# theivyzhang/droplet_visual_odometry

Measured on AMD Instinct MI355X. Metric: frames/sec (detect+match+pose) at 1280×720, 2000 feats; ATE vs reference, higher is better.
Workload: dtype u8/f32/f64

## Files before the change

### droplet_visual_odometry_amd/csrc/match.hip

```cpp
#include <algorithm>
#include <cfloat>
#include <climits>

#include "dvo_internal.h"

namespace dvo {
namespace {

typedef int v4i __attribute__((ext_vector_type(4)));
typedef int v8i __attribute__((ext_vector_type(8)));
typedef float v16f __attribute__((ext_vector_type(16)));
constexpr int kMWaves = 4, kMQB = 64 * kMWaves, kMStage = 64;
constexpr int kKeyBase = 1 << 20;

constexpr int kMChunks = 8;
constexpr int kMKs = 4;
typedef v16f acc_t;
__device__ __forceinline__ v4i expand_chunk(uint32_t bits, uint32_t base) {
    v4i r;
#pragma unroll
    for (int k = 0; k < 4; ++k) {
        const uint32_t L = (((bits >> (8 * k)) & 0xFu) * 0x00204081u) & 0x01010101u;
        const uint32_t H = (((bits >> (8 * k + 4)) & 0xFu) * 0x00204081u) & 0x01010101u;
        r[k] = (int)(base ^ (L << 3) ^ (H << 7));
    }
    return r;
}
constexpr uint32_t kExpQ = 0xAAAAAAAAu, kExpT = 0x22222222u;
__device__ __forceinline__ acc_t mfma_chunk(v4i a, v4i b, acc_t c) {
    const v8i A = {a[0], a[1], a[2], a[3], 0, 0, 0, 0}, B = {b[0], b[1], b[2], b[3], 0, 0, 0, 0};
    return __builtin_amdgcn_mfma_scale_f32_32x32x64_f8f6f4(A, B, c, 4, 4, 0, 0x7F7F7F7F, 0, 0x8B8B8B8B);
}
__device__ __forceinline__ int key_add(float a, float c) { return __float_as_int(a + c); }
__device__ __forceinline__ int key_value(int kbits) { return (int)__int_as_float(kbits); }
constexpr int kKeyNone = 0x7F000000;
constexpr int kChunkMask = kMChunks - 1;
__device__ __forceinline__ int key_old(int k) { return ((k >> 13) << 16) | (k & 8191); }

template <bool kFull>
__device__ __forceinline__ void nn_stage(const v4i* btc, int* cmin, const v4i (&A)[2][kMKs], int (&best)[2][16], int t0,
                                         int nt, int r, int h, int rowb, int nq) {
    const float rbf = (float)rowb;
    acc_t rb0, rb1;
#pragma unroll
    for (int g = 0; g < 16; ++g) {
        const int goff = (g & 3) + 8 * (g >> 2);
        rb0[g] = rbf + (float)goff;
        rb1[g] = rbf + (float)(32 + goff);
    }
#pragma unroll 1
    for (int tt = 0; tt < kMStage / 32; ++tt) {
        const int j = t0 + 32 * tt + r;
        const float cf = (float)(j < nt ? j : (1 << 30));
        acc_t acc0 = rb0, acc1 = rb1;
#pragma unroll
        for (int ks = 0; ks < kMKs; ++ks) {
            const v4i B = btc[(32 * tt + r) * kMChunks + ((2 * ks + h) ^ (r & kChunkMask))];
            acc0 = mfma_chunk(A[0][ks], B, acc0);
            acc1 = mfma_chunk(A[1][ks], B, acc1);
        }
        int cm = 0x7FFFFFFF;
#pragma unroll
        for (int g = 0; g < 16; ++g) {
            const int goff = (g & 3) + 8 * (g >> 2);
            best[0][g] = min(best[0][g], key_add(acc0[g], cf));
            best[1][g] = min(best[1][g], key_add(acc1[g], cf));
            int k0 = __float_as_int(acc0[g]), k1 = __float_as_int(acc1[g]);
            if (!kFull) {
                k0 = rowb - kKeyBase + goff < nq ? k0 : kKeyNone;
                k1 = rowb - kKeyBase + 32 + goff < nq ? k1 : kKeyNone;
            }
            cm = min(cm, min(k0, k1));
        }
        if (j < nt) atomicMin(&cmin[32 * tt + r], cm);
    }
}

struct NnOperands {
    const uint8_t* q0;
    const uint8_t* t0;
    int64_t stride;
    int nq_fix, nt_fix;
};

#ifndef DVO_MATCH_WAVES
#define DVO_MATCH_WAVES 1
#endif
__global__ __launch_bounds__(256) __attribute__((amdgpu_waves_per_eu(DVO_MATCH_WAVES)))
void nn_mfma_kernel(StreamParams P, NnOperands O, int pairs, int nqb, int tsplit) {
    __shared__ v4i bt[2][kMStage * kMChunks];
    __shared__ int colmin[2][kMStage];
    const int nwg = gridDim.x;
    const int L0 = (blockIdx.x & 7) * (nwg >> 3) + (blockIdx.x >> 3);
    const int L = L0 / tsplit, ts = L0 - L * tsplit;
    const int p = L / nqb, qb = L - p * nqb;
    if (p >= pairs) return;
    const int cap = P.plan.kp_cap;
    const int fp = pair_frame(P, p);
    const int nq = O.nq_fix >= 0 ? O.nq_fix : min(P.buf.nkp[fp], cap);
    const int nt = O.nt_fix >= 0 ? O.nt_fix : min(P.buf.nkp[fp + 1], cap);
    const int qbase = qb * kMQB;
    if (qbase >= nq) return;
    const int lane = threadIdx.x & 63, wid = threadIdx.x >> 6;
    const int r = lane & 31, h = lane >> 5;
    const uint4* XQ = reinterpret_cast<const uint4*>(O.q0 + fp * O.stride);
    const uint2* XT = reinterpret_cast<const uint2*>(O.t0 + fp * O.stride);
    int32_t* fwd = P.buf.nn + (int64_t)p * cap;
    int32_t* bwd = P.buf.nn + ((int64_t)P.nframes + p) * cap;
    const int qs = qbase + wid * 64;
    v4i A[2][kMKs];
    int best[2][16];
#pragma unroll
    for (int s2 = 0; s2 < 2; ++s2) {
        const int q = qs + 32 * s2 + r;
        const uint4 w0 = q < nq ? XQ[2 * (int64_t)q] : make_uint4(0, 0, 0, 0);
        const uint4 w1 = q < nq ? XQ[2 * (int64_t)q + 1] : make_uint4(0, 0, 0, 0);
        const uint32_t wd[8] = {w0.x, w0.y, w0.z, w0.w, w1.x, w1.y, w1.z, w1.w};
#pragma unroll
        for (int ks = 0; ks < kMKs; ++ks) {
            const int ch = 2 * ks + h;
            const uint32_t bits = wd[ch];
            A[s2][ks] = q < nq ? expand_chunk(bits, kExpQ) : (v4i){0, 0, 0, 0};
        }
#pragma unroll
        for (int g = 0; g < 16; ++g) best[s2][g] = 0x7FFFFFFF;
    }
    const int rowb = kKeyBase + qs + 4 * h;
    const bool full = qs + 64 <= nq;
    const int nst_all = (nt + kMStage - 1) / kMStage;
    const int st0 = (int)((int64_t)nst_all * ts / tsplit), nst = (int)((int64_t)nst_all * (ts + 1) / tsplit);
    const int tr = threadIdx.x >> 2, qd = threadIdx.x & 3;
    uint2 v;
    auto load_stage = [&](int st) { v = XT[(int64_t)min(st * kMStage + tr, nt - 1) * 4 + qd]; };
    auto store_stage = [&](int st, int b) {
        const bool in = st * kMStage + tr < nt;
        constexpr int kPer = kMChunks / 4;
#pragma unroll
        for (int c = 0; c < kPer; ++c) {
            const int ch = kPer * qd + c;
            const uint32_t bits = c == 0 ? v.x : v.y;
            bt[b][tr * kMChunks + (ch ^ (tr & kChunkMask))] = in ? expand_chunk(bits, kExpT) : (v4i){0, 0, 0, 0};
        }
        if (threadIdx.x < kMStage) colmin[b][threadIdx.x] = 0x7FFFFFFF;
    };
    if (st0 < nst) {
        load_stage(st0);
        store_stage(st0, 0);
    }
    __syncthreads();
    for (int st = st0; st < nst; ++st) {
        const int cur = (st - st0) & 1;
        if (st + 1 < nst) load_stage(st + 1);
        if (full) nn_stage<true>(bt[cur], colmin[cur], A, best, st * kMStage, nt, r, h, rowb, nq);
        else nn_stage<false>(bt[cur], colmin[cur], A, best, st * kMStage, nt, r, h, rowb, nq);
        if (st + 1 < nst) store_stage(st + 1, cur ^ 1);
        __syncthreads();
        const int t = st * kMStage + threadIdx.x;
        if (threadIdx.x < kMStage && t < nt && colmin[cur][threadIdx.x] != 0x7FFFFFFF)
            atomicMin(&bwd[t], key_old(key_value(colmin[cur][threadIdx.x])));
    }
#pragma unroll
    for (int s2 = 0; s2 < 2; ++s2)
#pragma unroll
        for (int g = 0; g < 16; ++g) {
            int vv = best[s2][g];
#pragma unroll
            for (int o = 1; o < 32; o <<= 1) vv = min(vv, __shfl_xor(vv, o));
            const int qr = qs + 32 * s2 + (g & 3) + 8 * (g >> 2) + 4 * h;
            if (r == g && qr < nq) {
                if (tsplit > 1) {
                    if (st0 < nst) atomicMin(&fwd[qr], key_old(key_value(vv) - qr));
                } else {
                    fwd[qr] = nt > 0 ? key_old(key_value(vv) - qr) : -1;
                }
            }
        }
}

constexpr int kXNT = 1024;
constexpr int kMaxSort = 8192;

__device__ int crosscheck_sort(const int32_t* fwd, const int32_t* bwd, int nq, int nt, int mode, uint32_t* keys,
                               int* scan_lds) {
    __shared__ int s_m;
    if (threadIdx.x == 0) s_m = 0;
    __syncthreads();
    if (mode == 2) {
        for (int q = threadIdx.x; q < nq; q += kXNT) keys[q] = 0xFFFFFFFFu;
        __syncthreads();
        for (int t = threadIdx.x; t < nt; t += kXNT) {
            int b = bwd[t];
            if (b < 0 || (b >> 16) > 256) continue;
            int q = b & 0xFFFF, d = b >> 16;
            atomicMin(&keys[q], ((uint32_t)d << 16) | (uint32_t)t);
        }
        __syncthreads();
        for (int q = threadIdx.x; q < nq; q += kXNT) {
            uint32_t k = keys[q];
            keys[kMaxSort + q] = k;
        }
        __syncthreads();
        for (int q = threadIdx.x; q < nq; q += kXNT) {
            uint32_t k = keys[kMaxSort + q];
            keys[q] = 0xFFFFFFFFu;
            if (k != 0xFFFFFFFFu) {
                int slot = atomicAdd(&s_m, 1);
                keys[slot] = ((k >> 16) << 16) | (uint32_t)q;
            }
        }
    } else {
        for (int q = threadIdx.x; q < nq; q += kXNT) {
            int f = fwd[q];
            if (f < 0 || (f >> 16) > 256) continue;
            int t = f & 0xFFFF;
            if (mode == 1 && (bwd[t] & 0xFFFF) != q) continue;
            int slot = atomicAdd(&s_m, 1);
            keys[slot] = ((uint32_t)(f >> 16) << 16) | (uint32_t)q;
        }
    }
    __syncthreads();
    const int m = s_m;
    int n2 = 1;
    while (n2 < m) n2 <<= 1;
    for (int i = m + threadIdx.x; i < n2; i += kXNT) keys[i] = 0xFFFFFFFFu;
    __syncthreads();
    for (int k = 2; k <= n2; k <<= 1)
        for (int j = k >> 1; j > 0; j >>= 1) {
            for (int i = threadIdx.x; i < n2; i += kXNT) {
                int ixj = i ^ j;
                if (ixj > i) {
                    uint32_t a = keys[i], b = keys[ixj];
                    bool up = (i & k) == 0;
                    if ((a > b) == up) {
                        keys[i] = b;
                        keys[ixj] = a;
                    }
                }
            }
            __syncthreads();
        }
    (void)scan_lds;
    return m;
}

__global__ __launch_bounds__(kXNT) void crosscheck_stream_kernel(StreamParams P, int mode) {
    __shared__ uint32_t keys[2 * kMaxSort];
    __shared__ int scan_lds[32];
    const int p = blockIdx.x;
    const int cap = P.plan.kp_cap;
    const int fp = pair_frame(P, p);
    const int nq = min(P.buf.nkp[fp], cap), nt = min(P.buf.nkp[fp + 1], cap);
    const int32_t* fwd = P.buf.nn + (int64_t)p * cap;
    const int32_t* bwd = P.buf.nn + ((int64_t)P.nframes + p) * cap;
    const int m = crosscheck_sort(fwd, bwd, nq, nt, mode, keys, scan_lds);
    const dvo_keypoint* ka = P.buf.kps + (int64_t)fp * cap;
    const dvo_keypoint* kb = P.buf.kps + (int64_t)(fp + 1) * cap;
    int32_t* mq = P.buf.mq + (int64_t)p * cap;
    int32_t* mt = P.buf.mt + (int64_t)p * cap;
    float* md = P.buf.md + (int64_t)p * cap;
    float* pts = P.buf.pts + (int64_t)p * cap * 4;
    for (int i = threadIdx.x; i < m; i += kXNT) {
        const uint32_t k = keys[i];
        const int q = k & 0xFFFF;
        const int t = mode == 2 ? (int)(keys[kMaxSort + q] & 0xFFFF) : (fwd[q] & 0xFFFF);
        mq[i] = q;
        mt[i] = t;
        md[i] = (float)(k >> 16);
        pts[4 * i + 0] = ka[q].x;
        pts[4 * i + 1] = ka[q].y;
        pts[4 * i + 2] = kb[t].x;
        pts[4 * i + 3] = kb[t].y;
    }
    if (threadIdx.x == 0) P.buf.nmatch[p] = m;
}

__global__ __launch_bounds__(kXNT) void crosscheck_pair_kernel(const int32_t* fwd, const int32_t* bwd, int nq, int nt,
                                                               int mode, dvo_dmatch* out, int* m_out) {
    __shared__ uint32_t best[kMaxSort];
    __shared__ int s_wave[kXNT / 64];
    __shared__ int s_carry;
    const int lane = threadIdx.x & 63, wid = threadIdx.x >> 6;
    if (mode == 2) {
        for (int q = threadIdx.x; q < nq; q += kXNT) best[q] = 0xFFFFFFFFu;
        __syncthreads();
        for (int t = threadIdx.x; t < nt; t += kXNT) {
            const int b = bwd[t];
            if (b < 0 || (b >> 16) > 256) continue;
            atomicMin(&best[b & 0xFFFF], ((uint32_t)(b >> 16) << 16) | (uint32_t)t);
        }
    }
    if (threadIdx.x == 0) s_carry = 0;
    __syncthreads();
    for (int q0 = 0; q0 < nq; q0 += kXNT) {
        const int q = q0 + threadIdx.x;
        bool keep = false;
        int t = 0, d = 0;
        if (q < nq) {
            if (mode == 2) {
                const uint32_t k = best[q];
                keep = k != 0xFFFFFFFFu;
                t = (int)(k & 0xFFFF);
                d = (int)(k >> 16);
            } else {
                const int f = fwd[q];
                if (f >= 0) {
                    t = f & 0xFFFF;
                    d = f >> 16;
                    keep = mode != 1 || (bwd[t] & 0xFFFF) == q;
                }
            }
        }
        const unsigned long long bal = __ballot(keep);
        if (lane == 0) s_wave[wid] = __popcll(bal);
        __syncthreads();
        int off = s_carry, tot = 0;
        for (int w = 0; w < kXNT / 64; ++w) {
            const int c = s_wave[w];
            off += w < wid ? c : 0;
            tot += c;
        }
        off += __builtin_amdgcn_mbcnt_hi((uint32_t)(bal >> 32), __builtin_amdgcn_mbcnt_lo((uint32_t)bal, 0u));
        if (keep) out[off] = dvo_dmatch{q, t, 0, (float)d};
        __syncthreads();
        if (threadIdx.x == 0) s_carry += tot;
        __syncthreads();
    }
    if (threadIdx.x == 0) *m_out = s_carry;
}

}

hipError_t launch_match(const StreamParams& P, int cross_check, hipStream_t s, hipEvent_t* ev, int tsplit) {
    const int pairs = stream_pairs(P);
    if (pairs < 1) return hipSuccess;
    mark(ev, 5, 0, s);
    const int cap = P.plan.kp_cap;
    hipError_t e = tsplit > 1
                       ? hipMemsetAsync(P.buf.nn, 0x7F, sizeof(int32_t) * 2 * (size_t)P.nframes * cap, s)
                       : hipMemsetAsync(P.buf.nn + (int64_t)P.nframes * cap, 0x7F,
                                        sizeof(int32_t) * (size_t)P.nframes * cap, s);
    if (e != hipSuccess) return e;
    const int nqb = (cap + kMQB - 1) / kMQB;
    const int nwg = ((pairs * nqb * tsplit + 7) / 8) * 8;
    const NnOperands O{P.buf.desc, P.buf.desc + (int64_t)cap * 32, (int64_t)cap * 32, -1, -1};
    hipLaunchKernelGGL(nn_mfma_kernel, dim3(nwg), dim3(256), 0, s, P, O, pairs, nqb, tsplit);
    hipLaunchKernelGGL(crosscheck_stream_kernel, dim3(pairs), dim3(kXNT), 0, s, P, cross_check);
    mark(ev, 5, 1, s);
    return hipGetLastError();
}

namespace {
int pair_cap(int nq, int nt) { return ((nq > nt ? nq : nt) + kMQB - 1) / kMQB * kMQB; }
}

size_t match_pair_work_size(int nq, int nt) { return 3 * (size_t)pair_cap(nq, nt) * sizeof(int32_t); }

hipError_t launch_match_pair(const uint8_t* d_q, int nq, const uint8_t* d_t, int nt, int cross_check, void* d_work,
                             dvo_dmatch* d_out, int* d_m, hipStream_t s) {
    const int cap = pair_cap(nq, nt);
    StreamParams P{};
    P.plan.kp_cap = cap;
    P.nframes = 2;
    P.pair_step = 1;
    P.buf.nn = static_cast<int32_t*>(d_work);
    int32_t* fwd = P.buf.nn;
    int32_t* bwd = P.buf.nn + 2 * (size_t)cap;
    hipError_t e = hipMemsetAsync(P.buf.nn, 0x7F, sizeof(int32_t) * 3 * (size_t)cap, s);
    if (e != hipSuccess) return e;
    const int nqb = cap / kMQB;
    const int nst = (nt + kMStage - 1) / kMStage;
    int tsplit = 1;
    while (tsplit < 16 && nqb * tsplit * 2 <= 256 && nst >= tsplit * 4) tsplit *= 2;
    const int nwg = ((nqb * tsplit + 7) / 8) * 8;
    const NnOperands O{d_q, d_t, 0, nq, nt};
    hipLaunchKernelGGL(nn_mfma_kernel, dim3(nwg), dim3(256), 0, s, P, O, 1, nqb, tsplit);
    hipLaunchKernelGGL(crosscheck_pair_kernel, dim3(1), dim3(kXNT), 0, s, fwd, bwd, nq, nt, cross_check, d_out, d_m);
    return hipGetLastError();
}

namespace {

struct KnnBytes {
    uint32_t *q, *t, *qn, *tn;
    int* rejected;
};

constexpr int kKnnQ = 256;
constexpr int kKnnTC = 64;
constexpr int kKnnWgPerCu = 3;
#ifndef DVO_KNN_G
#define DVO_KNN_G 2
#endif
constexpr int kKnnG = DVO_KNN_G;

template <int NORM>
__device__ __forceinline__ void dist_group(float& s, float a0, float a1, float a2, float a3, const float4 tv) {
    const float d0 = a0 - tv.x, d1 = a1 - tv.y, d2 = a2 - tv.z, d3 = a3 - tv.w;
    if constexpr (NORM == 0) {
        s += ((fabsf(d0) + fabsf(d1)) + fabsf(d2)) + fabsf(d3);
    } else {
        s += ((d0 * d0 + d1 * d1) + d2 * d2) + d3 * d3;
    }
}

template <int K>
__device__ __forceinline__ void knn_insert(float (&bd)[K], int (&bi)[K], float d, int j) {
    if (!(d < bd[K - 1])) return;
#pragma unroll
    for (int s = K - 1; s >= 0; --s) {
        if (bd[s] > d) {
            if (s > 0 && bd[s - 1] > d) {
                bd[s] = bd[s - 1];
                bi[s] = bi[s - 1];
            } else {
                bd[s] = d;
                bi[s] = j;
            }
        }
    }
}

template <int D, int NORM, int K>
__global__ __launch_bounds__(kKnnQ) void knn_float_kernel(const float* __restrict__ q, int nq,
                                                          const float* __restrict__ t, int nt, int range,
                                                          const int* __restrict__ u8_rejected,
                                                          float* __restrict__ odist, int32_t* __restrict__ oidx) {
    if (*u8_rejected == 0) return;
    constexpr int R = D / 4;
    static_assert(R % kKnnG == 0, "pipeline depth must divide the row");
    __shared__ float4 st[kKnnTC * R];
    const int qi = blockIdx.x * kKnnQ + threadIdx.x;
    const int qs = qi < nq ? qi : nq - 1;
    float qv[D];
    const float4* q4 = reinterpret_cast<const float4*>(q + (size_t)qs * D);
#pragma unroll
    for (int i = 0; i < R; ++i) {
        const float4 v = q4[i];
        qv[4 * i] = v.x;
        qv[4 * i + 1] = v.y;
        qv[4 * i + 2] = v.z;
        qv[4 * i + 3] = v.w;
    }
    float bd[K];
    int bi[K];
#pragma unroll
    for (int s = 0; s < K; ++s) {
        bd[s] = FLT_MAX;
        bi[s] = -1;
    }
    const int r0 = blockIdx.y * range, r1 = min(nt, r0 + range);
    for (int j0 = r0; j0 < r1; j0 += kKnnTC) {
        const int nj = min(r1 - j0, kKnnTC);
        const float4* src = reinterpret_cast<const float4*>(t + (size_t)j0 * D);
        if (j0 != r0) __syncthreads();
        for (int i = threadIdx.x; i < nj * R; i += kKnnQ) st[i] = src[i];
        __syncthreads();
        float4 cur[kKnnG];
#pragma unroll
        for (int e = 0; e < kKnnG; ++e) cur[e] = st[e];
        for (int j = 0; j < nj; ++j) {
            const float4* row = st + j * R;
            const float4* nrow = st + min(j + 1, nj - 1) * R;
            float s = 0.f;
#pragma unroll
            for (int g = 0; g < R; g += kKnnG) {
                float4 nxt[kKnnG];
                const float4* pf = g + kKnnG < R ? row + g + kKnnG : nrow;
#pragma unroll
                for (int e = 0; e < kKnnG; ++e) nxt[e] = pf[e];
                __builtin_amdgcn_sched_barrier(0);
#pragma unroll
                for (int e = 0; e < kKnnG; ++e) {
                    const int i = 4 * (g + e);
                    dist_group<NORM>(s, qv[i], qv[i + 1], qv[i + 2], qv[i + 3], cur[e]);
                }
#pragma unroll
                for (int e = 0; e < kKnnG; ++e) cur[e] = nxt[e];
            }
            knn_insert<K>(bd, bi, s, j0 + j);
        }
    }
    if (qi < nq) {
        const size_t o = ((size_t)blockIdx.y * nq + qi) * K;
#pragma unroll
        for (int s = 0; s < K; ++s) {
            odist[o + s] = bd[s];
            oidx[o + s] = bi[s];
        }
    }
}

__global__ __launch_bounds__(256) void knn_pack_u8_kernel(const float* __restrict__ xq, int nq,
                                                          const float* __restrict__ xt, int nt, int dim, int qblocks,
                                                          KnnBytes u8) {
    const bool side_q = (int)blockIdx.x < qblocks;
    const float* __restrict__ x = side_q ? xq : xt;
    const int n = side_q ? nq : nt;
    uint32_t* __restrict__ out = side_q ? u8.q : u8.t;
    uint32_t* __restrict__ norm = side_q ? u8.qn : u8.tn;
    int* __restrict__ rejected = u8.rejected;
    const int wpr = dim / 4;
    const int64_t id = (int64_t)(side_q ? blockIdx.x : blockIdx.x - qblocks) * 256 + threadIdx.x;
    const bool in = id < (int64_t)n * wpr;
    const float4 v = in ? reinterpret_cast<const float4*>(x)[id] : make_float4(0.f, 0.f, 0.f, 0.f);
    const float e[4] = {v.x, v.y, v.z, v.w};
    uint32_t word = 0, ss = 0;
    bool ok = true;
#pragma unroll
    for (int c = 0; c < 4; ++c) {
        ok &= e[c] >= 0.f && e[c] <= 255.f && e[c] == __builtin_rintf(e[c]);
        const uint32_t b = e[c] >= 0.f && e[c] <= 255.f ? (uint32_t)e[c] : 0u;
        word |= b << (8 * c);
        ss += b * b;
    }
    for (int o = 1; o < wpr; o <<= 1) ss += __shfl_xor(ss, o);
    if (in) {
        out[id] = word;
        if ((id & (wpr - 1)) == 0) norm[id / wpr] = ss;
    }
    if (__ballot(!ok) != 0 && (threadIdx.x & 63) == 0) atomicOr(rejected, 1);
}

#ifndef DVO_KNN_U8Q
#define DVO_KNN_U8Q 2
#endif
constexpr int kKnnU8Q = DVO_KNN_U8Q;
#ifndef DVO_KNN_RANGE_QB
#define DVO_KNN_RANGE_QB 256
#endif
constexpr int kKnnRangeQB = DVO_KNN_RANGE_QB;

template <int D, int NORM, int K>
__global__ __launch_bounds__(256) void knn_u8_kernel(const uint32_t* __restrict__ q, const uint32_t* __restrict__ qn,
                                                     int nq, const uint32_t* __restrict__ t,
                                                     const uint32_t* __restrict__ tn, int nt, int range,
                                                     const int* __restrict__ rejected, float* __restrict__ odist,
                                                     int32_t* __restrict__ oidx) {
    if (*rejected != 0) return;
    constexpr int W = D / 16;
    __shared__ uint4 st[kKnnTC * W];
    __shared__ uint32_t stn[kKnnTC];
    int qi[kKnnU8Q];
    uint4 qv[kKnnU8Q][W];
    uint32_t qnv[kKnnU8Q];
    float bd[kKnnU8Q][K];
    int bi[kKnnU8Q][K];
#pragma unroll
    for (int u = 0; u < kKnnU8Q; ++u) {
        qi[u] = blockIdx.x * (256 * kKnnU8Q) + 256 * u + threadIdx.x;
        const int qs = qi[u] < nq ? qi[u] : nq - 1;
        const uint4* q4 = reinterpret_cast<const uint4*>(q + (size_t)qs * (D / 4));
#pragma unroll
        for (int g = 0; g < W; ++g) qv[u][g] = q4[g];
        qnv[u] = qn[qs];
#pragma unroll
        for (int s2 = 0; s2 < K; ++s2) {
            bd[u][s2] = FLT_MAX;
            bi[u][s2] = -1;
        }
    }
    const int r0 = blockIdx.y * range, r1 = min(nt, r0 + range);
    for (int j0 = r0; j0 < r1; j0 += kKnnTC) {
        const int nj = min(r1 - j0, kKnnTC);
        const uint4* src = reinterpret_cast<const uint4*>(t + (size_t)j0 * (D / 4));
        if (j0 != r0) __syncthreads();
        for (int i = threadIdx.x; i < nj * W; i += 256) st[i] = src[i];
        if (threadIdx.x < nj) stn[threadIdx.x] = tn[j0 + threadIdx.x];
        __syncthreads();
        uint4 cur[W];
#pragma unroll
        for (int g = 0; g < W; ++g) cur[g] = st[g];
        for (int j = 0; j < nj; ++j) {
            uint4 nxt[W];
            const uint4* nrow = st + min(j + 1, nj - 1) * W;
#pragma unroll
            for (int g = 0; g < W; ++g) nxt[g] = nrow[g];
            const uint32_t tnj = stn[j];
            __builtin_amdgcn_sched_barrier(0);
#pragma unroll
            for (int u = 0; u < kKnnU8Q; ++u) {
                uint32_t acc = 0;
#pragma unroll
                for (int g = 0; g < W; ++g) {
                    if constexpr (NORM == 0) {
                        acc = __builtin_amdgcn_sad_u8(qv[u][g].x, cur[g].x, acc);
                        acc = __builtin_amdgcn_sad_u8(qv[u][g].y, cur[g].y, acc);
                        acc = __builtin_amdgcn_sad_u8(qv[u][g].z, cur[g].z, acc);
                        acc = __builtin_amdgcn_sad_u8(qv[u][g].w, cur[g].w, acc);
                    } else {
                        acc = __builtin_amdgcn_udot4(qv[u][g].x, cur[g].x, acc, false);
                        acc = __builtin_amdgcn_udot4(qv[u][g].y, cur[g].y, acc, false);
                        acc = __builtin_amdgcn_udot4(qv[u][g].z, cur[g].z, acc, false);
                        acc = __builtin_amdgcn_udot4(qv[u][g].w, cur[g].w, acc, false);
                    }
                }
                const uint32_t d = NORM == 0 ? acc : qnv[u] + tnj - 2u * acc;
                knn_insert<K>(bd[u], bi[u], (float)d, j0 + j);
            }
#pragma unroll
            for (int g = 0; g < W; ++g) cur[g] = nxt[g];
        }
    }
#pragma unroll
    for (int u = 0; u < kKnnU8Q; ++u)
        if (qi[u] < nq) {
            const size_t o = ((size_t)blockIdx.y * nq + qi[u]) * K;
#pragma unroll
            for (int s2 = 0; s2 < K; ++s2) {
                odist[o + s2] = bd[u][s2];
                oidx[o + s2] = bi[u][s2];
            }
        }
}

__device__ __forceinline__ bool knn_less(float da, int ia, float db, int ib) {
    return da < db || (da == db && ia < ib);
}

template <int K>
__device__ __forceinline__ void knn_merge2(float (&ad)[K], int (&ai)[K], const float (&bd)[K], const int (&bi)[K]) {
    float md[K];
    int mi[K];
    int pa = 0, pb = 0;
#pragma unroll
    for (int s = 0; s < K; ++s) {
        float da = FLT_MAX, db = FLT_MAX;
        int ia = INT_MAX, ib = INT_MAX;
#pragma unroll
        for (int u = 0; u < K; ++u) {
            if (u == pa) { da = ad[u]; ia = ai[u]; }
            if (u == pb) { db = bd[u]; ib = bi[u]; }
        }
        const bool ta = knn_less(da, ia, db, ib);
        md[s] = ta ? da : db;
        mi[s] = ta ? ia : ib;
        pa += ta;
        pb += !ta;
    }
#pragma unroll
    for (int s = 0; s < K; ++s) {
        ad[s] = md[s];
        ai[s] = mi[s];
    }
}

template <int K>
__global__ __launch_bounds__(256) void knn_merge_kernel(const float* __restrict__ pdist, const int32_t* __restrict__ pidx,
                                                        int nq, int ranges, float* __restrict__ odist,
                                                        int32_t* __restrict__ oidx) {
    const int qi = blockIdx.x * 4 + (threadIdx.x >> 6), lane = threadIdx.x & 63;
    if (qi >= nq) return;
    float bd[K];
    int bi[K];
#pragma unroll
    for (int s = 0; s < K; ++s) {
        bd[s] = FLT_MAX;
        bi[s] = INT_MAX;
    }
    for (int c = lane; c < ranges; c += 64) {
        const size_t o = ((size_t)c * nq + qi) * K;
        float cd[K];
        int ci[K];
#pragma unroll
        for (int s = 0; s < K; ++s) {
            const int i = pidx[o + s];
            cd[s] = i >= 0 ? pdist[o + s] : FLT_MAX;
            ci[s] = i >= 0 ? i : INT_MAX;
        }
        knn_merge2<K>(bd, bi, cd, ci);
    }
#pragma unroll
    for (int m = 1; m < 64; m <<= 1) {
        float od[K];
        int oi[K];
#pragma unroll
        for (int s = 0; s < K; ++s) {
            od[s] = __shfl_xor(bd[s], m, 64);
            oi[s] = __shfl_xor(bi[s], m, 64);
        }
        knn_merge2<K>(bd, bi, od, oi);
    }
    if (lane < K) {
        float d = bd[0];
        int i = bi[0];
#pragma unroll
        for (int s = 1; s < K; ++s)
            if (lane == s) {
                d = bd[s];
                i = bi[s];
            }
        odist[(size_t)qi * K + lane] = i == INT_MAX ? FLT_MAX : d;
        oidx[(size_t)qi * K + lane] = i == INT_MAX ? -1 : i;
    }
}

__global__ __launch_bounds__(256) void knn_pack_u8_batch_kernel(KnnBatchArgs a) {
    const int f = blockIdx.y;
    const int n = a.fstate[2 * f];
    const int wpr = a.dim / 4;
    const int64_t id = (int64_t)blockIdx.x * 256 + threadIdx.x, words = (int64_t)n * wpr;
    if ((int64_t)blockIdx.x * 256 >= words) return;
    const bool in = id < words;
    const float4* __restrict__ x = reinterpret_cast<const float4*>(a.desc + (size_t)f * a.cap * a.dim);
    const float4 v = in ? x[id] : make_float4(0.f, 0.f, 0.f, 0.f);
    const float e[4] = {v.x, v.y, v.z, v.w};
    uint32_t word = 0, ss = 0;
    bool ok = true;
#pragma unroll
    for (int c = 0; c < 4; ++c) {
        ok &= e[c] >= 0.f && e[c] <= 255.f && e[c] == __builtin_rintf(e[c]);
        const uint32_t b = e[c] >= 0.f && e[c] <= 255.f ? (uint32_t)e[c] : 0u;
        word |= b << (8 * c);
        ss += b * b;
    }
    for (int o = 1; o < wpr; o <<= 1) ss += __shfl_xor(ss, o);
    if (in) {
        a.bytes[(size_t)f * a.cap * wpr + id] = word;
        if ((id & (wpr - 1)) == 0) a.norms[(size_t)f * a.cap + id / wpr] = ss;
    }
    if (__ballot(!ok) != 0 && (threadIdx.x & 63) == 0) atomicOr(a.rejected + f, 1);
}

__device__ __forceinline__ size_t knn_batch_slot(const KnnBatchArgs& a, int p, int ranges, int c) {
    return (ranges == 1 ? (size_t)p : (size_t)p * ranges + c) * a.cap * 2;
}

template <int D>
__global__ __launch_bounds__(kKnnQ) void knn_float_batch_kernel(KnnBatchArgs a, int range) {
    constexpr int K = 2, R = D / 4;
    static_assert(R % kKnnG == 0, "pipeline depth must divide the row");
    __shared__ float4 st[kKnnTC * R];
    const int p = blockIdx.z, ranges = gridDim.y;
    const int nq = a.fstate[2 * p], nt = a.fstate[2 * p + 2];
    if ((int)(blockIdx.x * kKnnQ) >= nq) return;
    if (a.rejected && (a.rejected[p] | a.rejected[p + 1]) == 0) return;
    const int qi = blockIdx.x * kKnnQ + threadIdx.x;
    const size_t o = knn_batch_slot(a, p, ranges, blockIdx.y) + (size_t)qi * K;
    float* __restrict__ odist = ranges == 1 ? a.dist : a.pdist;
    int32_t* __restrict__ oidx = ranges == 1 ? a.idx : a.pidx;
    const int r0 = blockIdx.y * range, r1 = min(nt, r0 + range);
    if (r0 >= nt) {
        if (ranges == 1 && qi < nq) {
#pragma unroll
            for (int s = 0; s < K; ++s) {
                odist[o + s] = FLT_MAX;
                oidx[o + s] = -1;
            }
        }
        return;
    }
    const float* __restrict__ q = a.desc + (size_t)p * a.cap * D;
    const float* __restrict__ t = q + (size_t)a.cap * D;
    const int qs = qi < nq ? qi : nq - 1;
    float qv[D];
    const float4* q4 = reinterpret_cast<const float4*>(q + (size_t)qs * D);
#pragma unroll
    for (int i = 0; i < R; ++i) {
        const float4 v = q4[i];
        qv[4 * i] = v.x;
        qv[4 * i + 1] = v.y;
        qv[4 * i + 2] = v.z;
        qv[4 * i + 3] = v.w;
    }
    float bd[K];
    int bi[K];
#pragma unroll
    for (int s = 0; s < K; ++s) {
        bd[s] = FLT_MAX;
        bi[s] = -1;
    }
    for (int j0 = r0; j0 < r1; j0 += kKnnTC) {
        const int nj = min(r1 - j0, kKnnTC);
        const float4* src = reinterpret_cast<const float4*>(t + (size_t)j0 * D);
        if (j0 != r0) __syncthreads();
        for (int i = threadIdx.x; i < nj * R; i += kKnnQ) st[i] = src[i];
        __syncthreads();
        float4 cur[kKnnG];
#pragma unroll
        for (int e = 0; e < kKnnG; ++e) cur[e] = st[e];
        for (int j = 0; j < nj; ++j) {
            const float4* row = st + j * R;
            const float4* nrow = st + min(j + 1, nj - 1) * R;
            float s = 0.f;
#pragma unroll
            for (int g = 0; g < R; g += kKnnG) {
                float4 nxt[kKnnG];
                const float4* pf = g + kKnnG < R ? row + g + kKnnG : nrow;
#pragma unroll
                for (int e = 0; e < kKnnG; ++e) nxt[e] = pf[e];
                __builtin_amdgcn_sched_barrier(0);
#pragma unroll
                for (int e = 0; e < kKnnG; ++e) {
                    const int i = 4 * (g + e);
                    dist_group<0>(s, qv[i], qv[i + 1], qv[i + 2], qv[i + 3], cur[e]);
                }
#pragma unroll
                for (int e = 0; e < kKnnG; ++e) cur[e] = nxt[e];
            }
            knn_insert<K>(bd, bi, s, j0 + j);
        }
    }
    if (qi < nq) {
#pragma unroll
        for (int s = 0; s < K; ++s) {
            odist[o + s] = bd[s];
            oidx[o + s] = bi[s];
        }
    }
}

template <int D>
__global__ __launch_bounds__(256) void knn_u8_batch_kernel(KnnBatchArgs a, int range) {
    constexpr int K = 2, W = D / 16;
    __shared__ uint4 st[kKnnTC * W];
    const int p = blockIdx.z, ranges = gridDim.y;
    const int nq = a.fstate[2 * p], nt = a.fstate[2 * p + 2];
    if ((int)(blockIdx.x * (256 * kKnnU8Q)) >= nq) return;
    if ((a.rejected[p] | a.rejected[p + 1]) != 0) return;
    const size_t ob = knn_batch_slot(a, p, ranges, blockIdx.y);
    float* __restrict__ odist = ranges == 1 ? a.dist : a.pdist;
    int32_t* __restrict__ oidx = ranges == 1 ? a.idx : a.pidx;
    int qi[kKnnU8Q];
#pragma unroll
    for (int u = 0; u < kKnnU8Q; ++u) qi[u] = blockIdx.x * (256 * kKnnU8Q) + 256 * u + threadIdx.x;
    const int r0 = blockIdx.y * range, r1 = min(nt, r0 + range);
    if (r0 >= nt) {
        if (ranges == 1) {
#pragma unroll
            for (int u = 0; u < kKnnU8Q; ++u)
                if (qi[u] < nq) {
#pragma unroll
                    for (int s2 = 0; s2 < K; ++s2) {
                        odist[ob + (size_t)qi[u] * K + s2] = FLT_MAX;
                        oidx[ob + (size_t)qi[u] * K + s2] = -1;
                    }
                }
        }
        return;
    }
    const uint32_t* __restrict__ q = a.bytes + (size_t)p * a.cap * (D / 4);
    const uint32_t* __restrict__ t = q + (size_t)a.cap * (D / 4);
    uint4 qv[kKnnU8Q][W];
    float bd[kKnnU8Q][K];
    int bi[kKnnU8Q][K];
#pragma unroll
    for (int u = 0; u < kKnnU8Q; ++u) {
        const int qs = qi[u] < nq ? qi[u] : nq - 1;
        const uint4* q4 = reinterpret_cast<const uint4*>(q + (size_t)qs * (D / 4));
#pragma unroll
        for (int g = 0; g < W; ++g) qv[u][g] = q4[g];
#pragma unroll
        for (int s2 = 0; s2 < K; ++s2) {
            bd[u][s2] = FLT_MAX;
            bi[u][s2] = -1;
        }
    }
    for (int j0 = r0; j0 < r1; j0 += kKnnTC) {
        const int nj = min(r1 - j0, kKnnTC);
        const uint4* src = reinterpret_cast<const uint4*>(t + (size_t)j0 * (D / 4));
        if (j0 != r0) __syncthreads();
        for (int i = threadIdx.x; i < nj * W; i += 256) st[i] = src[i];
        __syncthreads();
        uint4 cur[W];
#pragma unroll
        for (int g = 0; g < W; ++g) cur[g] = st[g];
        for (int j = 0; j < nj; ++j) {
            uint4 nxt[W];
            const uint4* nrow = st + min(j + 1, nj - 1) * W;
#pragma unroll
            for (int g = 0; g < W; ++g) nxt[g] = nrow[g];
            __builtin_amdgcn_sched_barrier(0);
#pragma unroll
            for (int u = 0; u < kKnnU8Q; ++u) {
                uint32_t acc = 0;
#pragma unroll
                for (int g = 0; g < W; ++g) {
                    acc = __builtin_amdgcn_sad_u8(qv[u][g].x, cur[g].x, acc);
                    acc = __builtin_amdgcn_sad_u8(qv[u][g].y, cur[g].y, acc);
                    acc = __builtin_amdgcn_sad_u8(qv[u][g].z, cur[g].z, acc);
                    acc = __builtin_amdgcn_sad_u8(qv[u][g].w, cur[g].w, acc);
                }
                knn_insert<K>(bd[u], bi[u], (float)acc, j0 + j);
            }
#pragma unroll
            for (int g = 0; g < W; ++g) cur[g] = nxt[g];
        }
    }
#pragma unroll
    for (int u = 0; u < kKnnU8Q; ++u)
        if (qi[u] < nq) {
#pragma unroll
            for (int s2 = 0; s2 < K; ++s2) {
                odist[ob + (size_t)qi[u] * K + s2] = bd[u][s2];
                oidx[ob + (size_t)qi[u] * K + s2] = bi[u][s2];
            }
        }
}

__global__ __launch_bounds__(256) void knn_merge_batch_kernel(KnnBatchArgs a, int ranges, int range) {
    constexpr int K = 2;
    const int p = blockIdx.y;
    const int nq = a.fstate[2 * p], nt = a.fstate[2 * p + 2];
    const int qi = blockIdx.x * 4 + (threadIdx.x >> 6), lane = threadIdx.x & 63;
    if (qi >= nq) return;
    const size_t pb = (size_t)p * ranges * a.cap * K;
    float bd[K];
    int bi[K];
#pragma unroll
    for (int s = 0; s < K; ++s) {
        bd[s] = FLT_MAX;
        bi[s] = INT_MAX;
    }
    for (int c = lane; c < ranges && c * range < nt; c += 64) {
        const size_t o = pb + ((size_t)c * a.cap + qi) * K;
        float cd[K];
        int ci[K];
#pragma unroll
        for (int s = 0; s < K; ++s) {
            const int i = a.pidx[o + s];
            cd[s] = i >= 0 ? a.pdist[o + s] : FLT_MAX;
            ci[s] = i >= 0 ? i : INT_MAX;
        }
        knn_merge2<K>(bd, bi, cd, ci);
    }
#pragma unroll
    for (int m = 1; m < 64; m <<= 1) {
        float od[K];
        int oi[K];
#pragma unroll
        for (int s = 0; s < K; ++s) {
            od[s] = __shfl_xor(bd[s], m, 64);
            oi[s] = __shfl_xor(bi[s], m, 64);
        }
        knn_merge2<K>(bd, bi, od, oi);
    }
    if (lane < K) {
        const float d = lane == 0 ? bd[0] : bd[1];
        const int i = lane == 0 ? bi[0] : bi[1];
        const size_t o = ((size_t)p * a.cap + qi) * K + lane;
        a.dist[o] = i == INT_MAX ? FLT_MAX : d;
        a.idx[o] = i == INT_MAX ? -1 : i;
    }
}

template <int D, int NORM, int K>
hipError_t launch_knn_t(const float* d_q, int nq, const float* d_t, int nt, int ranges, const KnnBytes& u8,
                        float* d_part, int32_t* d_pidx, float* d_dist, int32_t* d_idx, hipStream_t s) {
    const int range = (nt + ranges - 1) / ranges;
    float* od = ranges == 1 ? d_dist : d_part;
    int32_t* oi = ranges == 1 ? d_idx : d_pidx;
    hipError_t e = hipMemsetAsync(u8.rejected, 0, sizeof(int), s);
    if (e != hipSuccess) return e;
    const int qblocks = (int)(((int64_t)nq * (D / 4) + 255) / 256), tblocks = (int)(((int64_t)nt * (D / 4) + 255) / 256);
    hipLaunchKernelGGL(knn_pack_u8_kernel, dim3(qblocks + tblocks), dim3(256), 0, s, d_q, nq, d_t, nt, D, qblocks, u8);
    hipLaunchKernelGGL((knn_u8_kernel<D, NORM, K>), dim3((nq + 256 * kKnnU8Q - 1) / (256 * kKnnU8Q), ranges), dim3(256), 0, s, u8.q, u8.qn, nq,
                       u8.t, u8.tn, nt, range, u8.rejected, od, oi);
    hipLaunchKernelGGL((knn_float_kernel<D, NORM, K>), dim3((nq + kKnnQ - 1) / kKnnQ, ranges), dim3(kKnnQ), 0, s, d_q,
                       nq, d_t, nt, range, u8.rejected, od, oi);
    if (ranges > 1)
        hipLaunchKernelGGL((knn_merge_kernel<K>), dim3((nq + 3) / 4), dim3(256), 0, s, d_part, d_pidx, nq, ranges,
                           d_dist, d_idx);
    return hipGetLastError();
}

template <int D, int NORM>
hipError_t launch_knn_k(int k, const float* d_q, int nq, const float* d_t, int nt, int ranges, const KnnBytes& u8,
                        float* d_part, int32_t* d_pidx, float* d_dist, int32_t* d_idx, hipStream_t s) {
    switch (k) {
        case 1: return launch_knn_t<D, NORM, 1>(d_q, nq, d_t, nt, ranges, u8, d_part, d_pidx, d_dist, d_idx, s);
        case 2: return launch_knn_t<D, NORM, 2>(d_q, nq, d_t, nt, ranges, u8, d_part, d_pidx, d_dist, d_idx, s);
        case 3: return launch_knn_t<D, NORM, 3>(d_q, nq, d_t, nt, ranges, u8, d_part, d_pidx, d_dist, d_idx, s);
        case 4: return launch_knn_t<D, NORM, 4>(d_q, nq, d_t, nt, ranges, u8, d_part, d_pidx, d_dist, d_idx, s);
        default: return hipErrorInvalidValue;
    }
}

}

int knn_ranges(int nq, int nt, int cus) {
    const int qblocks = (nq + kKnnRangeQB - 1) / kKnnRangeQB;
    int ranges = (cus * kKnnWgPerCu * 2) / qblocks;
    ranges = std::min(ranges, (nt + 15) / 16);
    ranges = std::max(ranges, 1);
    const int range = (nt + ranges - 1) / ranges;
    return (nt + range - 1) / range;
}

int knn_batch_ranges(int cap, int pairs, int cus) {
    const int64_t qblocks = (int64_t)((cap + kKnnRangeQB - 1) / kKnnRangeQB) * std::max(pairs, 1);
    int ranges = (int)std::min<int64_t>((cus * kKnnWgPerCu * 2) / qblocks, (cap + 15) / 16);
    ranges = std::max(ranges, 1);
    const int range = (cap + ranges - 1) / ranges;
    return (cap + range - 1) / range;
}

hipError_t launch_knn_batch(const KnnBatchArgs& a, int frames, int ranges, hipStream_t s) {
    const int pairs = frames - 1;
    if (pairs < 1) return hipSuccess;
    if ((a.dim != 128 && a.dim != 64) || a.cap < 1 || ranges < 1 || ranges > a.cap) return hipErrorInvalidValue;
    const int range = (a.cap + ranges - 1) / ranges;
    const bool bytes = a.dim == 128 && a.bytes != nullptr;
    const dim3 fgrid((a.cap + kKnnQ - 1) / kKnnQ, ranges, pairs);
    if (bytes) {
        hipError_t e = hipMemsetAsync(a.rejected, 0, sizeof(int32_t) * (size_t)frames, s);
        if (e != hipSuccess) return e;
        const int wblocks = (int)(((int64_t)a.cap * (a.dim / 4) + 255) / 256);
        hipLaunchKernelGGL(knn_pack_u8_batch_kernel, dim3(wblocks, frames), dim3(256), 0, s, a);
        hipLaunchKernelGGL(knn_u8_batch_kernel<128>, dim3((a.cap + 256 * kKnnU8Q - 1) / (256 * kKnnU8Q), ranges, pairs),
                           dim3(256), 0, s, a, range);
        hipLaunchKernelGGL(knn_float_batch_kernel<128>, fgrid, dim3(kKnnQ), 0, s, a, range);
    } else {
        KnnBatchArgs f = a;
        f.rejected = nullptr;
        if (a.dim == 128) hipLaunchKernelGGL(knn_float_batch_kernel<128>, fgrid, dim3(kKnnQ), 0, s, f, range);
        else hipLaunchKernelGGL(knn_float_batch_kernel<64>, fgrid, dim3(kKnnQ), 0, s, f, range);
    }
    if (ranges > 1)
        hipLaunchKernelGGL(knn_merge_batch_kernel, dim3((a.cap + 3) / 4, pairs), dim3(256), 0, s, a, ranges, range);
    return hipGetLastError();
}

size_t knn_bytes_size(int nq, int nt, int dim) { return (size_t)(nq + nt) * dim + 4 * (size_t)(nq + nt) + 16; }

hipError_t launch_knn_float(const float* d_q, int nq, const float* d_t, int nt, int dim, int k, int norm, int ranges,
                            void* d_bytes, float* d_part, int32_t* d_pidx, float* d_dist, int32_t* d_idx,
                            hipStream_t s) {
    if (nq <= 0 || nt <= 0) return hipSuccess;
    uint8_t* b = static_cast<uint8_t*>(d_bytes);
    KnnBytes u8;
    u8.q = reinterpret_cast<uint32_t*>(b);
    u8.t = reinterpret_cast<uint32_t*>(b + (size_t)nq * dim);
    u8.qn = reinterpret_cast<uint32_t*>(b + (size_t)(nq + nt) * dim);
    u8.tn = u8.qn + nq;
    u8.rejected = reinterpret_cast<int*>(u8.tn + nt);
    if (dim == 128)
        return norm == 0 ? launch_knn_k<128, 0>(k, d_q, nq, d_t, nt, ranges, u8, d_part, d_pidx, d_dist, d_idx, s)
                         : launch_knn_k<128, 1>(k, d_q, nq, d_t, nt, ranges, u8, d_part, d_pidx, d_dist, d_idx, s);
    if (dim == 64)
        return norm == 0 ? launch_knn_k<64, 0>(k, d_q, nq, d_t, nt, ranges, u8, d_part, d_pidx, d_dist, d_idx, s)
                         : launch_knn_k<64, 1>(k, d_q, nq, d_t, nt, ranges, u8, d_part, d_pidx, d_dist, d_idx, s);
    return hipErrorInvalidValue;
}

}
```

Measured before the change: 102,600.

## Simplify MFMA NN matching: cheaper bit expansion, precomputed row bias, higher occupancy

Replaces the multiply-and-mask nibble expansion in expand_chunk with a shift-and-mask that puts each descriptor bit into an FP4 lane. Precomputes per-row accumulator bias vectors once per kernel and encodes out-of-range query rows as a sentinel in the bias. This removes the full/partial template split and the per-element row check in the inner loop. The column-min reduction is split into two independent min chains to shorten dependency chains, and the waves-per-EU hint rises from 1 to 3 to allow more occupancy. Risks: the new bit layout and the sentinel bias must keep the same Hamming key semantics, and the occupancy hint may force register spills.

After: 103,300 (median of 6 runs). About the same (+0.7%).

```diff
diff --git a/droplet_visual_odometry_amd/csrc/match.hip b/droplet_visual_odometry_amd/csrc/match.hip
--- a/droplet_visual_odometry_amd/csrc/match.hip
+++ b/droplet_visual_odometry_amd/csrc/match.hip
@@ -19,11 +19,7 @@
 __device__ __forceinline__ v4i expand_chunk(uint32_t bits, uint32_t base) {
     v4i r;
 #pragma unroll
-    for (int k = 0; k < 4; ++k) {
-        const uint32_t L = (((bits >> (8 * k)) & 0xFu) * 0x00204081u) & 0x01010101u;
-        const uint32_t H = (((bits >> (8 * k + 4)) & 0xFu) * 0x00204081u) & 0x01010101u;
-        r[k] = (int)(base ^ (L << 3) ^ (H << 7));
-    }
+    for (int k = 0; k < 4; ++k) r[k] = (int)(base ^ ((bits << k) & 0x88888888u));
     return r;
 }
 constexpr uint32_t kExpQ = 0xAAAAAAAAu, kExpT = 0x22222222u;
@@ -37,42 +33,30 @@
 constexpr int kChunkMask = kMChunks - 1;
 __device__ __forceinline__ int key_old(int k) { return ((k >> 13) << 16) | (k & 8191); }
 
-template <bool kFull>
 __device__ __forceinline__ void nn_stage(const v4i* btc, int* cmin, const v4i (&A)[2][kMKs], int (&best)[2][16], int t0,
-                                         int nt, int r, int h, int rowb, int nq) {
-    const float rbf = (float)rowb;
-    acc_t rb0, rb1;
-#pragma unroll
-    for (int g = 0; g < 16; ++g) {
-        const int goff = (g & 3) + 8 * (g >> 2);
-        rb0[g] = rbf + (float)goff;
-        rb1[g] = rbf + (float)(32 + goff);
-    }
+                                         int nt, int r, int h, const acc_t (&rb)[2]) {
 #pragma unroll 1
     for (int tt = 0; tt < kMStage / 32; ++tt) {
         const int j = t0 + 32 * tt + r;
         const float cf = (float)(j < nt ? j : (1 << 30));
-        acc_t acc0 = rb0, acc1 = rb1;
+        acc_t acc0 = rb[0], acc1 = rb[1];
 #pragma unroll
         for (int ks = 0; ks < kMKs; ++ks) {
             const v4i B = btc[(32 * tt + r) * kMChunks + ((2 * ks + h) ^ (r & kChunkMask))];
             acc0 = mfma_chunk(A[0][ks], B, acc0);
             acc1 = mfma_chunk(A[1][ks], B, acc1);
         }
-        int cm = 0x7FFFFFFF;
-#pragma unroll
-        for (int g = 0; g < 16; ++g) {
-            const int goff = (g & 3) + 8 * (g >> 2);
+        int cm0 = 0x7FFFFFFF, cm1 = 0x7FFFFFFF;
+#pragma unroll
+        for (int g = 0; g < 16; g += 2) {
             best[0][g] = min(best[0][g], key_add(acc0[g], cf));
             best[1][g] = min(best[1][g], key_add(acc1[g], cf));
-            int k0 = __float_as_int(acc0[g]), k1 = __float_as_int(acc1[g]);
-            if (!kFull) {
-                k0 = rowb - kKeyBase + goff < nq ? k0 : kKeyNone;
-                k1 = rowb - kKeyBase + 32 + goff < nq ? k1 : kKeyNone;
-            }
-            cm = min(cm, min(k0, k1));
-        }
-        if (j < nt) atomicMin(&cmin[32 * tt + r], cm);
+            best[0][g + 1] = min(best[0][g + 1], key_add(acc0[g + 1], cf));
+            best[1][g + 1] = min(best[1][g + 1], key_add(acc1[g + 1], cf));
+            cm0 = min(min(cm0, __float_as_int(acc0[g])), __float_as_int(acc1[g]));
+            cm1 = min(min(cm1, __float_as_int(acc0[g + 1])), __float_as_int(acc1[g + 1]));
+        }
+        if (j < nt) atomicMin(&cmin[32 * tt + r], min(cm0, cm1));
     }
 }
 
@@ -84,7 +68,7 @@
 };
 
 #ifndef DVO_MATCH_WAVES
-#define DVO_MATCH_WAVES 1
+#define DVO_MATCH_WAVES 3
 #endif
 __global__ __launch_bounds__(256) __attribute__((amdgpu_waves_per_eu(DVO_MATCH_WAVES)))
 void nn_mfma_kernel(StreamParams P, NnOperands O, int pairs, int nqb, int tsplit) {
@@ -125,8 +109,14 @@
 #pragma unroll
         for (int g = 0; g < 16; ++g) best[s2][g] = 0x7FFFFFFF;
     }
-    const int rowb = kKeyBase + qs + 4 * h;
-    const bool full = qs + 64 <= nq;
+    acc_t rb[2];
+#pragma unroll
+    for (int s2 = 0; s2 < 2; ++s2)
+#pragma unroll
+        for (int g = 0; g < 16; ++g) {
+            const int row = qs + 32 * s2 + (g & 3) + 8 * (g >> 2) + 4 * h;
+            rb[s2][g] = row < nq ? (float)(kKeyBase + row) : __int_as_float(kKeyNone);
+        }
     const int nst_all = (nt + kMStage - 1) / kMStage;
     const int st0 = (int)((int64_t)nst_all * ts / tsplit), nst = (int)((int64_t)nst_all * (ts + 1) / tsplit);
     const int tr = threadIdx.x >> 2, qd = threadIdx.x & 3;
@@ -151,8 +141,7 @@
     for (int st = st0; st < nst; ++st) {
         const int cur = (st - st0) & 1;
         if (st + 1 < nst) load_stage(st + 1);
-        if (full) nn_stage<true>(bt[cur], colmin[cur], A, best, st * kMStage, nt, r, h, rowb, nq);
-        else nn_stage<false>(bt[cur], colmin[cur], A, best, st * kMStage, nt, r, h, rowb, nq);
+        nn_stage(bt[cur], colmin[cur], A, best, st * kMStage, nt, r, h, rb);
         if (st + 1 < nst) store_stage(st + 1, cur ^ 1);
         __syncthreads();
         const int t = st * kMStage + threadIdx.x;
```
